# Rorisis/Co-Occ

Hardware: AMD Instinct MI355X
Metric: samples/sec (6-cam frame + sweep -> occ+render), 200x200x16 grid (higher is better)
Workload: dtype f32 (split-f16 products, fp32 accumulate)

## Files before the change

### co_occ_amd/_lib.py

```python
import ctypes
import os
import threading
import time

import torch

_HERE = os.path.dirname(os.path.abspath(__file__))
LIB_PATH = os.path.join(_HERE, "libcoocc_hip.so")

c_int, c_float, c_void_p, c_size_t, c_int64 = (ctypes.c_int, ctypes.c_float, ctypes.c_void_p,
                                               ctypes.c_size_t, ctypes.c_int64)


class ConvDesc(ctypes.Structure):
    _fields_ = [(n, c_void_p) for n in ("in_", "w", "out", "scale", "bias", "res", "gather", "out_rows", "ws")] + \
               [("ws_floats", c_int64)] + \
               [(n, c_int) for n in ("M", "Cin", "Cout", "taps", "in_stride", "out_stride", "res_stride",
                                     "B", "Xi", "Yi", "Zi", "Xo", "Yo", "Zo", "ksize", "stride", "pad",
                                     "relu", "res_mode", "splitk", "tile_hint", "kx", "ky", "kz", "px", "py", "pz",
                                     "wgroup_rows", "mfma_dtype")] + [("alpha", ctypes.c_float), ("M_dev", c_void_p), ("gather_stride", c_int), ("out16", c_void_p), ("out16_stride", c_int), ("out_h2", c_int),
                                                                   ("out_h2_twin", c_void_p), ("tile_sem", c_void_p), ("tile_sem_ints", c_int),
                                                                  ("alpha_dev", c_void_p), ("sx", c_int), ("sy", c_int), ("sz", c_int)]


class SearchDesc(ctypes.Structure):
    _fields_ = [("cat4", c_void_p), ("pts", c_void_p), ("pts_rows", c_int), ("pts_stride", c_int)] + \
               [(n, c_int) for n in ("C", "X", "Y", "Z", "K", "fps_num", "max_cluster")] + \
               [("radius", ctypes.c_float), ("dist_thresh", ctypes.c_float), ("offsets", c_void_p), ("noff", c_int)] + \
               [(n, c_void_p) for n in ("lin", "counts", "near_img", "near_pts", "rows", "rows_p", "ws")] + \
               [("ws_bytes", ctypes.c_size_t), ("counts_host", c_void_p)]


P, I, F, Z, L = c_void_p, c_int, c_float, c_size_t, c_int64
SIGNATURES = {
    "coocc_last_error": (ctypes.c_char_p, []),
    "coocc_abi_version": (I, []),
    "coocc_device_cu_count": (I, [P]),
    "coocc_stream_create_cu_mask": (I, [P, I, P]),
    "coocc_stream_destroy": (I, [P]),
    "coocc_event_create": (I, [I, P]),
    "coocc_event_destroy": (I, [P]),
    "coocc_event_record": (I, [P, P]),
    "coocc_stream_wait_event": (I, [P, P]),
    "coocc_event_synchronize": (I, [P]),
    "coocc_event_query": (I, [P]),
    "coocc_event_elapsed_ms": (I, [P, P, P]),
    "coocc_ncdhw_to_ndhwc": (I, [P, P, I, I, I, I, I, P]),
    "coocc_rows_to_bf16": (I, [P, I, L, I, P, P]),
    "coocc_rows_to_h2": (I, [P, I, L, I, F, P, P]),
    "coocc_rows_to_h2_ex": (I, [P, I, L, I, F, P, P, P]),
    "coocc_rows_to_h2_gather": (I, [P, I, P, L, P, I, F, P, P]),
    "coocc_rows_to_f16": (I, [P, I, L, I, P, P]),
    "coocc_wino_input_h2": (I, [P, I, I, I, I, I, I, I, P, I, L, F, P]),
    "coocc_wino_input_h2_ex": (I, [P, I, I, I, I, I, I, I, P, I, L, F, P, P]),
    "coocc_ndhwc_to_ncdhw": (I, [P, P, I, I, I, I, I, P]),
    "coocc_fuser_prepare": (I, [P, P, P, P, P, I, I, I, P]),
    "coocc_fuser_prepare_rows": (I, [P, I, I, P, I, I, P, P, P, I, I, I, P]),
    "coocc_compact_flags": (I, [P, I, P, P, P, Z, P]),
    "coocc_compact_flags_ex": (I, [P, I, P, P, P, P, Z, P]),
    "coocc_lin_to_coords": (I, [P, I, I, I, I, P, P, P]),
    "coocc_furthest_point_sampling": (I, [I, I, I, P, P, P, P]),
    "coocc_fps_voxels_ws": (Z, [I, I, I]),
    "coocc_fps_voxels": (I, [P, I, I, I, I, I, P, P, Z, P]),
    "coocc_fps_voxels_pair": (I, [P, I, P, P, P, I, P, P, Z, I, I, I, I, P]),
    "coocc_ball_query": (I, [I, I, I, F, F, I, P, P, P, P]),
    "coocc_knn_topk": (I, [I, I, I, P, P, P, P, P]),
    "coocc_voxel_index_map": (I, [P, I, I, P, P]),
    "coocc_voxel_index_map_dev": (I, [P, I, P, I, P, P]),
    "coocc_fine_sample_voxel_dev": (I, [P, I, I, I, I, P, I, P, I, P, P, P, I, P]),
    "coocc_fine_sample_img_dev": (I, [P, I, I, I, I, P, P, L, P, P, I, I, P]),
    "coocc_fine_mlp_pre_dev": (I, [P, I, P, I, L, P, I, P, P, P, F, P, P, P, P, F, P, P, I, P, P]),
    "coocc_fine_fused": (I, [P, I, I, I, P, I, I, I, P, P, I, P, I, P, P, P, P, F, P, P, P, P, F, P, P, I, P, P, P]),
    "coocc_fine2_pack": (I, [P, P, I, P, P, P, P, P, P, P, P, P, P]),
    "coocc_fine2_h2": (I, [P, I, I, I, I, P, I, I, I, P, P, I, P, P, P, P, F, F, I, P, P, P, P]),
    "coocc_fine_sample_img_lin": (I, [P, I, I, I, I, P, P, I, I, I, P, P, I, I, P]),
    "coocc_scatter_fine_dev": (I, [P, L, P, I, I, I, P, P, I, I, I, F, P]),
    "coocc_scatter_fine_grouped": (I, [P, I, I, P, I, P, I, I, I, I, P, F, P, P]),
    "coocc_ball_query_voxels": (I, [I, F, F, I, I, I, I, P, P, P, P, P]),
    "coocc_knn_topk_voxels": (I, [I, I, I, I, I, I, P, P, P, P, I, P, P, P, P, P]),
    "coocc_knn_assign": (I, [I, I, I, I, F, P, P, P, P, P, P]),
    "coocc_knn_threshold": (I, [I, F, P, P, P, P]),
    "coocc_index_rows_i32": (I, [P, I, P, I, P, P]),
    "coocc_conv_pack_weights": (L, [P, I, I, I, I, P]),
    "coocc_conv_fwd": (I, [ctypes.POINTER(ConvDesc), P]),
    "coocc_fuser_search_ws": (Z, [ctypes.POINTER(SearchDesc)]),
    "coocc_fuser_search": (I, [ctypes.POINTER(SearchDesc), P, P]),
    "coocc_fuser_search_oneshot": (I, [I]),
    "coocc_lin_to_coords_dev": (I, [P, I, P, I, I, I, I, I, P, P]),
    "coocc_fps_voxels_pair_ok": (I, [I, I, I, I]),
    "coocc_fps_voxels_pair_dev": (I, [P, I, P, P, P, I, P, P, Z, I, P, I, I, I, I, I, P]),
    "coocc_knn_topk_voxels_dev": (I, [I, I, I, I, I, P, P, P, P, I, P, P, P, P, P, I, I, P]),
    "coocc_ball_query_voxels_dev": (I, [I, F, F, I, I, I, I, P, P, P, P, P, I, P]),
    "coocc_knn_assign_dev": (I, [I, I, I, I, F, P, P, P, P, P, P, I, I, P]),
# ... 331 lines not shown
```

### co_occ_amd/core.py

```python
import ctypes

import torch

from . import _lib
from ._lib import TIMER, ConvDesc, KernelTimer, call, ptr

_F32 = torch.float32


TILE_HINT = int(__import__("os").environ.get("COOCC_CONV_TILE", "0"))
CONV_V2 = int(__import__("os").environ.get("COOCC_CONV_V2", "1"))
WINO = int(__import__("os").environ.get("COOCC_WINO", "1"))
WINO_MIN_ROWS = int(__import__("os").environ.get("COOCC_WINO_MIN_ROWS", "8192"))
CONV_PERSIST = __import__("os").environ.get("COOCC_CONV_PERSIST", "1") != "0"
ZTRIM = __import__("os").environ.get("COOCC_ZTRIM", "1") != "0"
WINO_TILE = int(__import__("os").environ.get("COOCC_WINO_TILE", "4"))
CONV_DTYPE = __import__("os").environ.get("COOCC_CONV_DTYPE", "f32")
CONV_ENGINE = __import__("os").environ.get("COOCC_CONV_ENGINE", "h2")
H2_WINO_SCALE = {2: 0.5, 3: 0.25, 4: 0.125}
H2_DIRECT = __import__("os").environ.get("COOCC_H2_DIRECT", "1") != "0"
INKERNEL_REDUCE = __import__("os").environ.get("COOCC_INKERNEL_REDUCE", "0") != "0"
H2_DIRECT_MIN_FLOPS = float(__import__("os").environ.get("COOCC_H2_MIN_FLOPS", "5e7"))


# ... 295 lines not shown
            return None
        return self._cached(("h2", ztrim), lambda: self._h2_layout(self._padded(self._taps(ztrim).double())))

    @staticmethod
    def _wino_G(tile):
        if tile == 2:
            return torch.tensor([[1., 0., 0.], [.5, .5, .5], [.5, -.5, .5], [0., 0., 1.]], dtype=torch.float64)
        if tile == 3:
            return torch.tensor([[1, 0, 0], [-2 / 9, 2 / 9, -2 / 9], [1 / 9, 2 / 9, 4 / 9], [-8 / 9, -4 / 9, -2 / 9], [0, 0, 1]],
                                dtype=torch.float64)
        return torch.tensor([[1, 0, 0], [1 / 3, 1 / 3, 1 / 3], [-1 / 3, 1 / 3, -1 / 3], [-16 / 15, -8 / 15, -4 / 15],
                             [1 / 15, -2 / 15, 4 / 15], [0, 0, 1]], dtype=torch.float64)

    def _wino_U(self, tile):
        G = self._wino_G(tile)
        w = self._w_raw.double().view(self.Cout, self.Cin, 3, 3, self.wino_kz)
        return torch.einsum("pa,qb,ncabz->pqncz", G, G, w).reshape(G.shape[0] ** 2, self.Cout, self.Cin, self.wino_kz)

    def wino_h2_pack(self, tile):
        return self._cached(("wino_h2", tile), lambda: torch.stack(
            [self._h2_layout(self._padded(u)) for u in self._wino_U(tile)], 0))

    def wino_pack(self, tile):
        def build():
            return torch.stack([lib_pack("coocc_conv_pack_weights", u, self.Cout, self.Cin, self.wino_kz, 0)
                                for u in self._wino_U(tile).float().contiguous()], 0)
        return self._cached(("wino", tile), build)


BF16_PRECONVERT = __import__("os").environ.get("COOCC_BF16_PRECONVERT", "1") != "0"
ZSHARE = __import__("os").environ.get("COOCC_BF16_ZSHARE", "1") != "0"

_stream_bufs = {}


def stream_buffer(device, kind, n, dtype=_F32, zero=False):
    key = (device.index, _lib.stream(device).value or 0, kind)
    t = _stream_bufs.get(key)
    if t is None or t.numel() < n:
        t = _stream_bufs[key] = (torch.zeros if zero else torch.empty)(n, device=device, dtype=dtype)
    return t


def stream_scratch(device, stream):
    h = stream.cuda_stream
    return [t for (d, s, _), t in _stream_bufs.items() if d == device.index and s == h]


def _wino_buffer(device, kind, nfloats):
    return stream_buffer(device, kind, nfloats, zero=True)


def scratch(device, kind, nfloats):
    return stream_buffer(device, "s:" + kind, nfloats)


def tile_sem(device, n=4096):
    return stream_buffer(device, "sem", n, torch.int32, zero=True)


def workspace(device, nfloats=64 << 20):
    return stream_buffer(device, "ws", nfloats)


def _lcm(a, b):
    import math
    return a * b // math.gcd(a, b)


# ... 375 lines not shown
```

### co_occ_amd/csrc/layout.hip

```cpp
#include <stdarg.h>
#include <stdlib.h>

#include "common.h"

typedef float f32x4 __attribute__((ext_vector_type(4)));

static thread_local char g_err[512] = "";

int coocc_set_error(int code, const char* fmt, ...) {
  va_list ap;
  va_start(ap, fmt);
  vsnprintf(g_err, sizeof(g_err), fmt, ap);
  va_end(ap);
  return code;
}

extern "C" const char* coocc_last_error(void) { return g_err; }
extern "C" int coocc_abi_version(void) { return 1; }

#define TV 64
#define TC 128

__global__ __launch_bounds__(256) void k_ncdhw_to_ndhwc(const float* __restrict__ src,
                                                         float* __restrict__ dst, int C, int V,
// ... 418 lines not shown
  if (cnt) {
    if (cnt[0] <= small_m || cnt[1] <= small_m) return;
    n = min(n, cnt[which]);
  }
  int i = blockIdx.x * blockDim.x + threadIdx.x;
  if (i >= n) return;
  int l = lin[i];
  int z = l % Z; l /= Z;
  int y = l % Y; l /= Y;
  int x = l % X; int b = l / X;
  if (xyz) { xyz[i * 3 + 0] = (float)x; xyz[i * 3 + 1] = (float)y; xyz[i * 3 + 2] = (float)z; }
  if (bxyz) { bxyz[i * 4 + 0] = b; bxyz[i * 4 + 1] = x; bxyz[i * 4 + 2] = y; bxyz[i * 4 + 3] = z; }
}

extern "C" int coocc_lin_to_coords(const int32_t* lin, int n, int X, int Y, int Z, float* xyz, int64_t* bxyz,
                                   void* stream) {
  COOCC_CHECK_ARG(lin && n >= 0 && X > 0 && Y > 0 && Z > 0, "lin_to_coords: bad args");
  if (n == 0) return COOCC_OK;
  hipLaunchKernelGGL(k_lin_to_coords, dim3(cdiv(n, 256)), dim3(256), 0, as_stream(stream), lin, n, X, Y, Z, xyz, bxyz,
                     (const int32_t*)nullptr, 0, 0);
  COOCC_LAUNCH_CHECK("k_lin_to_coords");
  return COOCC_OK;
}

extern "C" int coocc_lin_to_coords_dev(const int32_t* lin, int n_cap, const int32_t* cnt, int which, int small_m, int X, int Y, int Z,
                                       float* xyz, void* stream) {
  COOCC_CHECK_ARG(lin && xyz && cnt && n_cap > 0 && (unsigned)which < 2u && X > 0 && Y > 0 && Z > 0, "lin_to_coords_dev: bad args");
  hipLaunchKernelGGL(k_lin_to_coords, dim3(cdiv(n_cap, 256)), dim3(256), 0, as_stream(stream), lin, n_cap, X, Y, Z, xyz, (int64_t*)nullptr,
                     cnt, which, small_m);
  COOCC_LAUNCH_CHECK("k_lin_to_coords");
  return COOCC_OK;
}

extern "C" int coocc_device_cu_count(int* n) {
  COOCC_CHECK_ARG(n, "device_cu_count: null");
  int dev = 0;
  COOCC_HIP(hipGetDevice(&dev));
  hipDeviceProp_t prop;
  COOCC_HIP(hipGetDeviceProperties(&prop, dev));
  *n = prop.multiProcessorCount;
  return COOCC_OK;
}

extern "C" int coocc_stream_create_cu_mask(const uint32_t* mask_host, int nwords, void** stream_out) {
  COOCC_CHECK_ARG(mask_host && nwords > 0 && stream_out, "stream_create_cu_mask: bad args");
  hipStream_t s = nullptr;
  COOCC_HIP(hipExtStreamCreateWithCUMask(&s, (uint32_t)nwords, mask_host));
  *stream_out = (void*)s;
  return COOCC_OK;
}

extern "C" int coocc_stream_destroy(void* stream) {
  COOCC_CHECK_ARG(stream, "stream_destroy: null");
  COOCC_HIP(hipStreamDestroy(as_stream(stream)));
  return COOCC_OK;
}

extern "C" int coocc_event_create(int flags, void** event_out) {
  COOCC_CHECK_ARG(event_out && (flags & ~3) == 0, "event_create: bad args");
  hipEvent_t e = nullptr;
  COOCC_HIP(hipEventCreateWithFlags(&e, hipEventDisableSystemFence | ((flags & 1) ? 0u : hipEventDisableTiming) |
                                            ((flags & 2) ? hipEventBlockingSync : 0u)));
  *event_out = (void*)e;
  return COOCC_OK;
}
extern "C" int coocc_event_destroy(void* event) {
// ... 32 lines not shown
```

### co_occ_amd/csrc/search.hip

```cpp
#include <stdlib.h>
#include <string.h>

#include <atomic>

#include "common.h"

__global__ __launch_bounds__(256) void k_gather_xyz(const float* __restrict__ xyz, const int32_t* __restrict__ idx, int m,
                                                     float* __restrict__ out, const int32_t* __restrict__ cnt, int small_m) {
  if (cnt && (cnt[0] <= small_m || cnt[1] <= small_m)) return;
  const int i = blockIdx.x * blockDim.x + threadIdx.x;
  if (i >= m) return;
  const int s = idx[i];
  out[i * 3 + 0] = xyz[s * 3 + 0]; out[i * 3 + 1] = xyz[s * 3 + 1]; out[i * 3 + 2] = xyz[s * 3 + 2];
}

struct SearchWs {
  uint8_t* flags;
  int32_t* cws;
  float* xyz;
  int32_t* maps;
  int32_t* rep[2];
  float* rep_xyz[2];
  float* val[2];
  int32_t* nn[2];
// ... 74 lines not shown
  SRC(coocc_voxel_index_map_dev(lin_img, V, cnt, V, map_img, stream));
  SRC(coocc_voxel_index_map_dev(lin_pts, V, cnt + 1, V, map_pts, stream));
  if (!(sdiag & 1)) {
    const int rc = coocc_fps_voxels_pair_dev(lin_pts, 1, w.rep[0], w.fps[0], lin_img, 0, w.rep[1], w.fps[1], w.fps_bytes, V, cnt, m, X, Y, Z, m,
                                             stream);
    if (rc == 2) return coocc_set_error(COOCC_EINVAL, "fuser_search: the paired FPS refused a grid it had accepted");
    SRC(rc);
  }
  auto direction = [&](int dd, const int32_t* lin_q, int wq, const float* xyz_q, const int32_t* map_q, int wk, const float* xyz_k,
                       const int32_t* map_k, int32_t* near) -> int {
    if (sdiag & 2) return COOCC_OK;
    hipLaunchKernelGGL(k_gather_xyz, dim3(cdiv(m, 256)), dim3(256), 0, as_stream(stream), xyz_q, w.rep[dd], m, w.rep_xyz[dd], cnt, m);
    COOCC_LAUNCH_CHECK("k_gather_xyz");
    SRC(coocc_knn_topk_voxels_dev(m, K, X, Y, Z, w.rep[dd], lin_q, map_k, d->offsets, d->noff, w.rep_xyz[dd], xyz_k, w.val[dd], w.nn[dd], cnt,
                                  wk, m, stream));
    SRC(coocc_ball_query_voxels_dev(m, 0.f, d->radius, d->max_cluster, X, Y, Z, w.rep[dd], lin_q, map_q, w.group[dd], cnt, m, stream));
    SRC(coocc_knn_assign_dev(m, K, d->max_cluster, V, d->dist_thresh, w.val[dd], w.nn[dd], w.group[dd], w.winner[dd], near, cnt, wq, m, stream));
    return COOCC_OK;
  };
  SRC(direction(1, lin_img, 0, xyz_img, map_img, 1, xyz_pts, map_pts, d->near_pts));
  for (int k = 0; k < K && !(sdiag & 2); ++k)
    SRC(coocc_index_rows_i32_dev(K == 1 ? lin_pts : lin_img, K == 1 ? 1 : 0, d->near_pts, k, 0, V, d->rows_p + (size_t)k * V, cnt, m, stream));
  SRC(direction(0, lin_pts, 1, xyz_pts, map_pts, 0, xyz_img, map_img, d->near_img));
  for (int k = 0; k < K && !(sdiag & 2); ++k)
    SRC(coocc_index_rows_i32_dev(lin_img, 0, d->near_img, k, 1, V, d->rows + (size_t)k * V, cnt, m, stream));
  return COOCC_OK;
}

extern "C" int coocc_fuser_search(coocc_search_desc* d, void* stream, void* side_stream) {
  COOCC_CHECK_ARG(d && d->cat4 && d->pts && d->lin && d->counts && d->rows && d->rows_p && d->near_img && d->near_pts && d->ws &&
                      d->offsets && d->counts_host, "fuser_search: null pointer");
  COOCC_CHECK_ARG(d->C > 0 && d->X > 0 && d->Y > 0 && d->Z > 0 && d->K >= 1 && d->K <= 8 && d->fps_num > 0 && d->max_cluster > 0 &&
                      d->noff > 0, "fuser_search: bad sizes");
  COOCC_CHECK_ARG(stream != side_stream && side_stream, "fuser_search: needs a second stream for the img <- pts direction");
  const int V = d->X * d->Y * d->Z, K = d->K, C = d->C;
  SearchWs w = carve((char*)d->ws, V, K, d->fps_num, d->max_cluster, d->X, d->Y, d->Z);
  COOCC_CHECK_ARG(d->ws_bytes >= w.total, "fuser_search: workspace smaller than coocc_fuser_search_ws()");
  hipStream_t s0 = as_stream(stream), s1 = as_stream(side_stream);
  static const int sdiag = [] { const char* e = getenv("COOCC_SEARCH_DIAG_SKIP"); return e ? atoi(e) : 0; }();
  int32_t* lin_img = d->lin;
  int32_t* lin_pts = d->lin + V;

  SRC(coocc_fuser_prepare_rows(d->cat4, 1, 4 * C, d->pts, d->pts_rows, d->pts_stride, d->cat4, w.flags, w.flags + V, 1, C, V, stream));
  SRC(coocc_compact_flags(w.flags, V, lin_img, d->counts, w.cws, (size_t)(V / 1024 + 2) * 4, stream));
  SRC(coocc_compact_flags(w.flags + V, V, lin_pts, d->counts + 1, w.cws + (V / 1024 + 2), (size_t)(V / 1024 + 2) * 4, stream));
  if (oneshot_setting() && d->fps_num >= K && coocc_fps_voxels_pair_ok(V, d->X, d->Y, d->Z)) {
    const bool read = !((sdiag & 4) && d->counts_host[0] > 0);
    volatile int32_t* pin = read ? pinned_counts() : nullptr;
    if (read && !pin) return coocc_set_error(COOCC_ENOMEM, "fuser_search: no pinned host memory for the voxel counts");
    hipEvent_t got = nullptr;
    if (read) {
      static const bool fence = [] { const char* e = getenv("COOCC_SEARCH_COUNT_FENCE"); return e && e[0] == '1'; }();
      pin[0] = pin[1] = -1;
      COOCC_HIP(hipMemcpyAsync((void*)pin, d->counts, 8, hipMemcpyDeviceToHost, s0));
      COOCC_HIP(hipEventCreateWithFlags(&got, hipEventBlockingSync | hipEventDisableTiming | (fence ? 0u : hipEventDisableSystemFence)));
      if (hipEventRecord(got, s0) != hipSuccess) {
        (void)hipEventDestroy(got);
        return coocc_set_error(COOCC_EHIP, "fuser_search: recording the count event failed");
      }
    }
    const int rc = search_enqueue_dev(d, w, V, stream, sdiag);
    if (read) {
      const hipError_t e2 = hipEventSynchronize(got);
      (void)hipEventDestroy(got);
      if (e2 != hipSuccess) return coocc_set_error(COOCC_EHIP, "fuser_search: waiting for the voxel counts failed: %s", hipGetErrorString(e2));
      if (pin[0] < 0 || pin[1] < 0) {
        COOCC_HIP(hipStreamSynchronize(s0));
        if (pin[0] < 0 || pin[1] < 0) return coocc_set_error(COOCC_EHIP, "fuser_search: the voxel counts did not reach the host");
// ... 23 lines not shown
  int32_t* map_img = w.maps;
  int32_t* map_pts = w.maps + V;
  SRC(coocc_voxel_index_map(lin_img, Ni, V, map_img, stream));
  SRC(coocc_voxel_index_map(lin_pts, Np, V, map_pts, stream));

  const int pair_rc = (sdiag & 1) ? COOCC_OK
                                  : coocc_fps_voxels_pair(lin_pts, Np, w.rep[0], w.fps[0], lin_img, Ni, w.rep[1], w.fps[1], w.fps_bytes, d->X, d->Y,
                                                          d->Z, d->fps_num, stream);
  if (pair_rc != COOCC_OK && pair_rc != 2) return pair_rc;
  const bool paired = pair_rc == COOCC_OK;
  hipEvent_t fork = nullptr, join = nullptr;
  COOCC_HIP(hipEventCreateWithFlags(&fork, hipEventDisableTiming | hipEventDisableSystemFence));
  if (hipEventCreateWithFlags(&join, hipEventDisableTiming | hipEventDisableSystemFence) != hipSuccess) {
    (void)hipEventDestroy(fork);
    return coocc_set_error(COOCC_EHIP, "fuser_search: hipEventCreate failed");
  }
  bool forked = false;
  auto finish = [&](int rc) -> int {
    if (forked) {
      if (hipEventRecord(join, s1) != hipSuccess || hipStreamWaitEvent(s0, join, 0) != hipSuccess) {
        if (rc == COOCC_OK) rc = coocc_set_error(COOCC_EHIP, "fuser_search: joining the side stream failed");
      }
    }
    (void)hipEventDestroy(fork);
    (void)hipEventDestroy(join);
    return rc;
  };
#define SRF(call)                                \
  do {                                           \
    int rc__ = (call);                           \
    if (rc__ != COOCC_OK) return finish(rc__);   \
  } while (0)
  void* side_q = paired ? stream : side_stream;
  if (!paired) {
    if (hipEventRecord(fork, s0) != hipSuccess || hipStreamWaitEvent(s1, fork, 0) != hipSuccess)
      return finish(coocc_set_error(COOCC_EHIP, "fuser_search: forking the side stream failed"));
    forked = true;
  }

  auto direction = [&](int dd, void* st, const int32_t* lin_q, int Q, const float* xyz_q, const int32_t* map_q, int Nk,
                       const float* xyz_k, const int32_t* map_k, int32_t* near) -> int {
    if (sdiag & 2) return COOCC_OK;
    if (!paired) SRC(coocc_fps_voxels(lin_q, Q, d->X, d->Y, d->Z, d->fps_num, w.rep[dd], w.fps[dd], w.fps_bytes, st));
    hipLaunchKernelGGL(k_gather_xyz, dim3(cdiv(d->fps_num, 256)), dim3(256), 0, as_stream(st), xyz_q, w.rep[dd], d->fps_num, w.rep_xyz[dd],
                       (const int32_t*)nullptr, 0);
    COOCC_LAUNCH_CHECK("k_gather_xyz");
    SRC(coocc_knn_topk_voxels(d->fps_num, Nk, K, d->X, d->Y, d->Z, w.rep[dd], lin_q, map_k, d->offsets, d->noff, w.rep_xyz[dd], xyz_k,
                              w.val[dd], w.nn[dd], st));
    SRC(coocc_ball_query_voxels(d->fps_num, 0.f, d->radius, d->max_cluster, d->X, d->Y, d->Z, w.rep[dd], lin_q, map_q, w.group[dd], st));
    SRC(coocc_knn_assign(d->fps_num, K, d->max_cluster, Q, d->dist_thresh, w.val[dd], w.nn[dd], w.group[dd], w.winner[dd], near, st));
    return COOCC_OK;
  };
  SRF(direction(1, side_q, lin_img, Ni, xyz_img, map_img, Np, xyz_pts, map_pts, d->near_pts));
  for (int k = 0; k < K && !(sdiag & 2); ++k)
    SRF(coocc_index_rows_i32(K == 1 ? lin_pts : lin_img, K == 1 ? Np : Ni, d->near_pts + (size_t)k * Ni, Ni, d->rows_p + (size_t)k * V, side_q));
  SRF(direction(0, stream, lin_pts, Np, xyz_pts, map_pts, Ni, xyz_img, map_img, d->near_img));
  for (int k = 0; k < K && !(sdiag & 2); ++k)
    SRF(coocc_index_rows_i32(lin_img, Ni, d->near_img + (size_t)k * Np, Np, d->rows + (size_t)k * V, stream));
#undef SRF
  return finish(COOCC_OK);
}
```

### co_occ_amd/fuser.py

```python
import torch
from torch import nn

from . import _lib, streams
from ._lib import call, ptr
from . import core as _core_mod
from .core import PackCache, PackedConv, Rows, conv_rows, gather_conv_rows
from .registry import FUSION_LAYERS

_I32, _F32, _I64 = torch.int32, torch.float32, torch.int64


_side = {}


def _side_stream(dev, cur, which=0):
    key = (dev.index, cur.cuda_stream, which)
    if key not in _side:
        _side[key] = streams.side_stream_for(cur, which) or torch.cuda.Stream(device=dev, priority=getattr(cur, "priority", 0))
    return _side[key]


FPS_HIGH_PRIORITY = __import__("os").environ.get("COOCC_FPS_HIGH_PRIORITY", "0") != "0"
_fps_hi = {}
FPS_MAX_BUCKETS = 8 * 1024
# ... 311 lines not shown
                base, nbase = (lin_pts, Np) if K == 1 else (lin_img, Ni)
                for k in range(K):
                    call("coocc_index_rows_i32", ptr(base), nbase, ptr(sr.near_pts[k]), Ni, ptr(sr.rows_p[k]))
                sr.done_side = streams.new_event()
                sr.done_side.record()
            sr.near_img = _fps_nn_xyz(xyz_pts, xyz_img, q_lin=lin_pts if vox else None, k_lin=lin_img if vox else None, grid=vox,
                                      which=0, home=cur, **kw)
            sr.rows = slot.rows[:, :Np] if slot is not None else torch.empty(K, Np, device=dev, dtype=_I32)
            for k in range(K):
                call("coocc_index_rows_i32", ptr(lin_img), Ni, ptr(sr.near_img[k]), Np, ptr(sr.rows[k]))
            sr.keep = (xyz, lin, img, pts)
        elif Np or Ni:
            raise IndexError("BiFuser_N: one modality has no non-empty voxel (the reference fails on empty keys)")
        sr.done_main = streams.new_event()
        sr.done_main.record()
        return sr

    def search_native(self, pts_voxel_feats, slot):
        import ctypes
        X, Y, Z = slot.grid
        dev = slot.cat4.device
        pts_r = _as_rows_view(pts_voxel_feats)
        B = pts_r.B if pts_r is not None else pts_voxel_feats.shape[0]
        if B != 1 or (X + 3) // 4 * ((Y + 3) // 4) * ((Z + 7) // 8) > FPS_MAX_BUCKETS:
            return self.search(slot.img_rows().as_ncdhw(), pts_voxel_feats, slot=slot)
        d, _, host, _ = slot.native_desc()
        if pts_r is not None:
            d.pts, d.pts_rows, d.pts_stride = pts_r.t.data_ptr() + 4 * pts_r.coff, 1, pts_r.stride
            keep = pts_r.t
        else:
            keep = pts_voxel_feats.float().contiguous()
            d.pts, d.pts_rows, d.pts_stride = keep.data_ptr(), 0, 0
        cur = torch.cuda.current_stream(dev)
        side = _side_stream(dev, cur)
        rc = _lib.load().coocc_fuser_search(ctypes.byref(d), ctypes.c_void_p(cur.cuda_stream), ctypes.c_void_p(side.cuda_stream))
        if rc == 1:
            return self.search(slot.img_rows().as_ncdhw(), pts_voxel_feats, slot=slot)
        _lib.check(rc)
        Ni, Np = int(host[0]), int(host[1])
        self.last_counts = (Ni, Np)
        K, V = self.knum, slot.V
        sr = SearchResult(Rows(slot.cat4, 1, X, Y, Z, 4 * self.in_channels), slot.lin[0, :Ni], slot.lin[1, :Np])
        sr.slot = slot
        sr.near_img = slot.near[0, :K * Np].view(K, Np)
        sr.near_pts = slot.near[1, :K * Ni].view(K, Ni)
        sr.rows, sr.rows_p = slot.rows[:, :Np], slot.rows_p[:, :Ni]
        sr.keep = (keep,)
        sr.done_main = streams.new_event()
        sr.done_main.record()
        sr.done_side = sr.done_main
        return sr

    def finish(self, sr):
        cat4 = sr.cat4.t
        dev = cat4.device
        C = self.in_channels
        cur = torch.cuda.current_stream(dev)
        packs = self._packed()
        sr.done_main.wait(cur)
        for t in sr.tensors():
            t.record_stream(cur)
        if sr.rows is not None and sr.slot is not None:
            sr.done_side.wait(cur)
            self.finish_static(sr.slot)
            self.last_near = (sr.near_img, sr.near_pts)
        elif sr.rows is not None:
            sr.done_side.wait(cur)
            h2 = self._g1_h2(cat4, packs)
# ... 114 lines not shown
```

### co_occ_amd/serving.py

```python
import collections
import os
import threading
import time
from concurrent.futures import ThreadPoolExecutor

import torch

from . import core, graph as cg, streams as cstreams_

CAM_KEYS = ("rots", "trans", "intrins", "post_rots", "post_trans", "bda")


def _tensors_of(obj):
    if torch.is_tensor(obj):
        yield obj
    elif isinstance(obj, dict):
        for v in obj.values():
            yield from _tensors_of(v)
    elif isinstance(obj, (list, tuple)):
        for v in obj:
            yield from _tensors_of(v)


class Ticket:

    __slots__ = ("pipe", "index", "slot", "frame", "search", "out", "done", "copy", "events", "fallback", "ready", "pts_vol", "stream")

    def __init__(self, pipe, index, slot, frame, copy):
        self.pipe, self.index, self.slot, self.frame, self.copy = pipe, index, slot, frame, copy
        self.search = self.out = self.done = self.events = self.pts_vol = self.stream = None
        self.fallback = False
        self.ready = cstreams_.new_event()
        self.ready.record(torch.cuda.current_stream(pipe.dev))

    def result(self, wait=True):
        self.pipe._issue_through(self.index)
        if wait:
            self.done.synchronize()
            core.check_h2_overflow()
        return self.out


_DIAG_SKIP = int(os.environ.get("COOCC_SERVING_DIAG_SKIP", "0"))
SLOT_WAIT_HOST = os.environ.get("COOCC_SLOT_WAIT", "host") != "device"


def _clone_frame_item(v):
    if torch.is_tensor(v):
        return v.detach().clone()
    if isinstance(v, (list, tuple)):
        return type(v)(_clone_frame_item(x) for x in v)
    return v


class ServingPipeline:

    def __init__(self, model, example, slots=6, dense_streams=3, ahead=0, render=None, search_priority=0, after_replay=None,
                 time_dense=False, after_done=None):
        assert not model.training, "ServingPipeline serves the eval-mode (folded-BN) path"
        self.model = model
        pts = example.get("pts")
        if pts is None:
            with torch.no_grad():
                pts = model.extract_pts_feat(example["points"])[0]
        self.dev = dev = pts.device
        _, _, X, Y, Z = pts.shape
        self.grid = (X, Y, Z)
        self.render = (X >= 100 and Y >= 100 and Z >= 8 and model.use_rendering) if render is None else render
        self.n = n = max(1, int(slots))
        self.ndense = max(1, min(int(dense_streams), max(1, n - 1)))
        most = max(1, n - self.ndense) if n > 1 else 1
        self.ahead = most if ahead <= 0 else max(1, min(int(ahead), most))
        self.after_replay, self.after_done, self.time_dense = after_replay, after_done, time_dense
        self.dense_streams = [torch.cuda.Stream(device=dev) for _ in range(self.ndense)]
        self.search_streams = [torch.cuda.Stream(device=dev, priority=search_priority) for _ in range(n)]
        self.slots = [cg.make_slot(model, self.grid, dev) for _ in range(n)]
        self.static = [self._make_static(example) for _ in range(n)]
        self.slot_done = [None] * n
        self.graphs = [None] * n
        self.tpool = ThreadPoolExecutor(self.ahead)
        self.fallbacks = 0
        self.dense_ev = []
        self.trace = [] if os.environ.get("COOCC_SERVING_TRACE", "0") == "1" else None
        self._lock = threading.Lock()
        self._pending = collections.deque()
        self._queue = collections.deque()
        self._submitted = self._issued = 0
        self._issued_of_slot = [0] * n
        self._dispatched_of_slot = [0] * n
        self._last_sr = [None] * n
        self._example = {k: _clone_frame_item(v) for k, v in example.items()}
        self.recaptures = 0
        self._capture(example)
        self._watch = core.WeightWatch(model)

    def _make_static(self, fr):
        dev = self.dev
        cams = fr.get("cams")
        tr = fr["transform"]
        size = tr[-1]
        size = tuple(int(v[0]) if torch.is_tensor(v) else int(v) for v in size)
        st = dict(img_feats=[torch.empty_like(fr["img_feats"][0], device=dev)],
                  cams=tuple(torch.empty_like(t, device=dev) for t in cams) if cams is not None else None,
                  transform=tuple(torch.empty_like(t, device=dev) if torch.is_tensor(t) else t for t in tr[:-1]) + (size,),
                  gemo=None)
        if cams is None:
            st["gemo"] = torch.empty_like(fr["gemo"], device=dev) if fr.get("gemo") is not None else None
        return st

    def _copy_in(self, k, fr):
        st = self.static[k]
        st["img_feats"][0].copy_(fr["img_feats"][0], non_blocking=True)
        if st["cams"] is not None:
            for d, s in zip(st["cams"], fr["cams"]):
                d.copy_(s, non_blocking=True)
        for d, s in zip(st["transform"][:-1], fr["transform"][:-1]):
            if torch.is_tensor(d):
                d.copy_(s, non_blocking=True)
        if st["gemo"] is not None:
            st["gemo"].copy_(fr["gemo"], non_blocking=True)

    def _mark(self, t, tag):
        if self.trace is not None:
            self.trace.append((t.index, tag, time.perf_counter()))

    def _search(self, t):
        k, fr = t.slot, t.frame
        torch.cuda.set_device(self.dev)
        self._mark(t, "search_begin")
        st = self.search_streams[k]
        with torch.cuda.stream(st), torch.no_grad():
            t.ready.wait(st)
            if self.slot_done[k] is not None:
                if SLOT_WAIT_HOST:
                    self.slot_done[k].synchronize()
                else:
                    self.slot_done[k].wait(st)
            if self.time_dense:
                e0 = cstreams_.new_event(timing=True)
                e0.record()
            for v in _tensors_of(fr):
                if v.is_cuda:
                    v.record_stream(st)
            diag = _DIAG_SKIP if t.index >= 0 else 0
            if not diag & 1:
                self._copy_in(k, fr)
            pts = fr.get("pts")
            if pts is None:
                pts = self.model.extract_pts_feat(fr["points"])[0]
            t.pts_vol = pts
            self._mark(t, "search_native")
            slot = self.slots[k]
            if diag & 6 and fr.get("depth") is not None and self._last_sr[k] is not None:
                if not diag & 2:
                    self.model.img_view_transformer.lift_splat(fr["depth"], fr["ctx"], cams=fr["cams"], out=slot.img_rows())
                if not diag & 4:
                    sr = self.model.occ_fuser.search_native(pts, slot)
                else:
                    sr = self._last_sr[k]
                    sr.done_main = cstreams_.new_event()
                    sr.done_main.record()
                    sr.done_side = sr.done_main
            elif fr.get("depth") is not None:
                sr = cg.search_into_slot(self.model, slot, fr["depth"], fr["ctx"], fr["cams"], pts)
                self._last_sr[k] = sr
            else:
                vol = fr["img_voxel_feats"]
                slot.img_rows().as_ncdhw().copy_(vol)
                sr = self.model.occ_fuser.search_native(pts, slot) if cg.NATIVE_SEARCH else \
                    self.model.occ_fuser.search(slot.img_rows().as_ncdhw(), pts, slot=slot)
            if self.time_dense:
                if sr.done_side is not None:
                    sr.done_side.wait(st)
                e1 = cstreams_.new_event(timing=True)
                e1.record()
                t.events = (e0, e1)
        self._mark(t, "search_end")
        return sr

    def _capture(self, example):
        for k in range(self.n):
            t = Ticket(self, -1, k, example, False)
            sr = self._search(t)
            ds = self.dense_streams[k % self.ndense]
            sr.done_main.wait(ds)
            if sr.done_side is not None:
                sr.done_side.wait(ds)
            self.graphs[k] = cg.DenseGraph(self.model, self.slots[k], self.static[k], ds, render=self.render).capture()
        torch.cuda.synchronize(self.dev)
        core.check_h2_overflow()

    def submit(self, frame, copy=False):
        if self._watch.changed():
            self._recapture()
        with self._lock:
            i = self._submitted
            self._submitted += 1
            t = Ticket(self, i, i % self.n, frame, copy)
            self._pending.append(t)
        self._pump()
        return t

    def _pump(self, block_until=None):
        while True:
            with self._lock:
                while self._pending and len(self._queue) < self.ahead:
                    t = self._pending[0]
                    if self._dispatched_of_slot[t.slot] > self._issued_of_slot[t.slot]:
                        break
                    self._pending.popleft()
                    self._dispatched_of_slot[t.slot] += 1
                    self._mark(t, "dispatch")
                    t.search = self.tpool.submit(self._search, t)
                    self._queue.append(t)
                head = self._queue[0] if self._queue else None
            if head is None:
                return
            must = block_until is not None and self._issued <= block_until
            if not (must or head.search.done()):
                return
            sr = head.search.result()
            self._mark(head, "issue_begin")
            self._issue(head, sr)
            self._mark(head, "issue_end")
            with self._lock:
                self._queue.popleft()
                self._issued += 1
                self._issued_of_slot[head.slot] += 1

    def _issue_through(self, index):
        if self._issued <= index:
            self._pump(block_until=index)
        assert self._issued > index

    def _issue(self, t, sr):
        k = t.slot
        ds = self.dense_streams[k % self.ndense]
        sr.done_main.wait(ds)
        if sr.done_side is not None:
            sr.done_side.wait(ds)
        with torch.cuda.stream(ds), torch.no_grad():
            if self.time_dense:
                e0 = cstreams_.new_event(timing=True)
                e0.record()
            g = self.graphs[k]
            if g.fits(sr.counts):
                out = g.replay()
            else:
                self.fallbacks += 1
                t.fallback = True
                st = self.static[k]
                vf = self.model.occ_fuser(self.slots[k].img_rows().as_ncdhw(), t.pts_vol, search=sr)
                cam_geo = None
                if self.render and st["cams"] is not None:
                    cam_geo = self.model.img_view_transformer._camera_mats(*st["cams"])
                    cam_geo = (cam_geo[0].reshape(-1, cam_geo[0].shape[-1]),) + tuple(cam_geo[1:])
                out = self.model.decode(vf, st["gemo"], st["img_feats"], st["transform"], self.render, cam_geo=cam_geo)
            if self.time_dense:
                e1 = cstreams_.new_event(timing=True)
                e1.record()
                self.dense_ev.append((e0, e1, t.index, t.events))
            if t.copy:
                out = {kk: (v.clone() if torch.is_tensor(v) else (v.as_ncdhw().clone() if isinstance(v, core.Rows) else v))
                       for kk, v in out.items()}
            if self.after_replay is not None:
                self.after_replay(out)
            ev = cstreams_.new_event(blocking=True)
            ev.record()
        self.slot_done[k] = ev
        if self.after_done is not None:
            self.after_done(out, ev)
        t.out, t.done, t.stream = out, ev, ds
        t.frame = t.pts_vol = None
# ... 36 lines not shown
```

### include/coocc_hip.h

```cpp
#ifndef COOCC_HIP_H
#define COOCC_HIP_H

#include <stddef.h>
#include <stdint.h>

#ifdef __cplusplus
extern "C" {
#endif

#define COOCC_OK 0
#define COOCC_EINVAL (-1)
#define COOCC_EHIP (-2)
#define COOCC_ENOMEM (-3)

const char* coocc_last_error(void);
int coocc_abi_version(void);

int coocc_device_cu_count(int* n);
int coocc_stream_create_cu_mask(const uint32_t* mask_host, int nwords, void** stream_out);
int coocc_stream_destroy(void* stream);

int coocc_event_create(int flags, void** event_out);
int coocc_event_destroy(void* event);
int coocc_event_record(void* event, void* stream);
int coocc_stream_wait_event(void* stream, void* event);
int coocc_event_synchronize(void* event);
int coocc_event_query(void* event);
int coocc_event_elapsed_ms(void* start, void* stop, float* ms);


int coocc_ncdhw_to_ndhwc(const float* src, float* dst, int B, int C, int V, int dst_stride,
                         int dst_coff, void* stream);
int coocc_ndhwc_to_ncdhw(const float* src, float* dst, int B, int C, int V, int src_stride,
                         int src_coff, void* stream);

int coocc_fuser_prepare(const float* img, const float* pts, float* cat4, uint8_t* flag_img,
                        uint8_t* flag_pts, int B, int C, int V, void* stream);
int coocc_fuser_prepare_rows(const float* img, int img_rows, int img_stride, const float* pts, int pts_rows,
                             int pts_stride, float* cat4, uint8_t* flag_img, uint8_t* flag_pts, int B, int C, int V,
                             void* stream);

int coocc_compact_flags(const uint8_t* flags, int total, int32_t* lin, int32_t* count, void* ws,
                        size_t ws_bytes, void* stream);
int coocc_compact_flags_ex(const uint8_t* flags, int total, int32_t* lin, int32_t* count, int32_t* map, void* ws,
                           size_t ws_bytes, void* stream);
int coocc_lin_to_coords(const int32_t* lin, int n, int X, int Y, int Z, float* xyz, int64_t* bxyz,
                        void* stream);


int coocc_furthest_point_sampling(int b, int n, int m, const float* points, float* temp,
                                  int32_t* idx, void* stream);

size_t coocc_fps_voxels_ws(int X, int Y, int Z);
int coocc_fps_voxels(const int32_t* lin, int n, int X, int Y, int Z, int m, int32_t* idx, void* ws,
                     size_t ws_bytes, void* stream);
int coocc_fps_voxels_pair(const int32_t* lin0, int n0, int32_t* idx0, void* ws0, const int32_t* lin1, int n1, int32_t* idx1,
                          void* ws1, size_t ws_bytes_each, int X, int Y, int Z, int m, void* stream);

int coocc_ball_query(int b, int n, int m, float min_radius, float max_radius, int nsample,
                     const float* new_xyz, const float* xyz, int32_t* idx, void* stream);

#define COOCC_SEARCH_SMALL 1
typedef struct coocc_search_desc {
  float* cat4;
  const float* pts;
  int pts_rows, pts_stride;
  int C, X, Y, Z, K;
  int fps_num, max_cluster;
  float radius, dist_thresh;
  const uint32_t* offsets;
  int noff;
  int32_t* lin;
  int32_t* counts;
  int32_t* near_img;
  int32_t* near_pts;
  int32_t* rows;
  int32_t* rows_p;
  void* ws;
  size_t ws_bytes;
  int32_t* counts_host;
// ... 513 lines not shown
```

Before: 272.3.

## Run search on dense-stream lanes and batch frame input copies into one kernel

```diff
diff --git a/co_occ_amd/_lib.py b/co_occ_amd/_lib.py
--- a/co_occ_amd/_lib.py
+++ b/co_occ_amd/_lib.py
@@ -30,6 +30,12 @@
                [(n, c_void_p) for n in ("lin", "counts", "near_img", "near_pts", "rows", "rows_p", "ws")] + \
                [("ws_bytes", ctypes.c_size_t), ("counts_host", c_void_p)]
 
+
+class CopyItem(ctypes.Structure):
+    _fields_ = [("dst", c_void_p), ("src", c_void_p), ("bytes", ctypes.c_size_t)]
+
+
+COPY_MANY_MAX = 16
 
 P, I, F, Z, L = c_void_p, c_int, c_float, c_size_t, c_int64
 SIGNATURES = {
@@ -59,6 +65,7 @@
     "coocc_compact_flags": (I, [P, I, P, P, P, Z, P]),
     "coocc_compact_flags_ex": (I, [P, I, P, P, P, P, Z, P]),
     "coocc_lin_to_coords": (I, [P, I, I, I, I, P, P, P]),
+    "coocc_copy_many": (I, [P, I, P]),
     "coocc_furthest_point_sampling": (I, [I, I, I, P, P, P, P]),
     "coocc_fps_voxels_ws": (Z, [I, I, I]),
     "coocc_fps_voxels": (I, [P, I, I, I, I, I, P, P, Z, P]),
diff --git a/co_occ_amd/core.py b/co_occ_amd/core.py
--- a/co_occ_amd/core.py
+++ b/co_occ_amd/core.py
@@ -351,9 +351,25 @@
 ZSHARE = __import__("os").environ.get("COOCC_BF16_ZSHARE", "1") != "0"
 
 _stream_bufs = {}
+_scratch_ns = __import__("threading").local()
+
+
+class scratch_space:
+
+    def __init__(self, name):
+        self.name = name
+
+    def __enter__(self):
+        self.prev = getattr(_scratch_ns, "name", "")
+        _scratch_ns.name = self.name
+        return self
+
+    def __exit__(self, *exc):
+        _scratch_ns.name = self.prev
 
 
 def stream_buffer(device, kind, n, dtype=_F32, zero=False):
+    kind = getattr(_scratch_ns, "name", "") + kind
     key = (device.index, _lib.stream(device).value or 0, kind)
     t = _stream_bufs.get(key)
     if t is None or t.numel() < n:
diff --git a/co_occ_amd/csrc/layout.hip b/co_occ_amd/csrc/layout.hip
--- a/co_occ_amd/csrc/layout.hip
+++ b/co_occ_amd/csrc/layout.hip
@@ -474,6 +474,73 @@
   return COOCC_OK;
 }
 
+constexpr int COPY_THREADS = 256;
+constexpr unsigned long long COPY_CHUNK = 16384;
+constexpr unsigned long long COPY_MAX_BLOCKS = 4096;
+
+struct CopyTable {
+  char* dst[COOCC_COPY_MANY_MAX];
+  const char* src[COOCC_COPY_MANY_MAX];
+  unsigned long long bytes[COOCC_COPY_MANY_MAX];
+  unsigned first[COOCC_COPY_MANY_MAX + 1];
+  unsigned long long chunk;
+  int n;
+};
+
+__global__ __launch_bounds__(COPY_THREADS) void k_copy_many(const CopyTable t) {
+  const unsigned b = blockIdx.x;
+  int i = 0;
+#pragma unroll
+  for (int k = 1; k < COOCC_COPY_MANY_MAX; ++k)
+    if (k < t.n && b >= t.first[k]) i = k;
+  const unsigned long long off = (unsigned long long)(b - t.first[i]) * t.chunk;
+  const unsigned long long total = t.bytes[i];
+  if (off >= total) return;
+  const unsigned long long len = total - off < t.chunk ? total - off : t.chunk;
+  char* d = t.dst[i] + off;
+  const char* s = t.src[i] + off;
+  const uintptr_t al = (uintptr_t)d | (uintptr_t)s;
+  unsigned long long done = 0;
+  if ((al & 15) == 0) {
+    const unsigned long long nv = len >> 4;
+    for (unsigned long long v = threadIdx.x; v < nv; v += COPY_THREADS) ((uint4*)d)[v] = ((const uint4*)s)[v];
+    done = nv << 4;
+  }
+  if ((al & 3) == 0) {
+    const unsigned long long nw = (len - done) >> 2;
+    for (unsigned long long w = threadIdx.x; w < nw; w += COPY_THREADS) ((uint32_t*)(d + done))[w] = ((const uint32_t*)(s + done))[w];
+    done += nw << 2;
+  }
+  for (unsigned long long k = done + threadIdx.x; k < len; k += COPY_THREADS) d[k] = s[k];
+}
+
+extern "C" int coocc_copy_many(const coocc_copy_item* items, int n, void* stream) {
+  COOCC_CHECK_ARG(items && n >= 1 && n <= COOCC_COPY_MANY_MAX, "copy_many: 1 .. %d items per call", COOCC_COPY_MANY_MAX);
+  CopyTable t;
+  unsigned long long total = 0;
+  for (int i = 0; i < n; ++i) {
+    COOCC_CHECK_ARG(items[i].bytes == 0 || (items[i].dst && items[i].src), "copy_many: null pointer in item %d", i);
+    total += items[i].bytes;
+  }
+  if (total == 0) return COOCC_OK;
+  t.chunk = COPY_CHUNK * ((total / COPY_MAX_BLOCKS + COPY_CHUNK - 1) / COPY_CHUNK);
+  if (t.chunk < COPY_CHUNK) t.chunk = COPY_CHUNK;
+  unsigned nblk = 0;
+  for (int i = 0; i < COOCC_COPY_MANY_MAX; ++i) {
+    const bool on = i < n;
+    t.dst[i] = on ? (char*)items[i].dst : nullptr;
+    t.src[i] = on ? (const char*)items[i].src : nullptr;
+    t.bytes[i] = on ? (unsigned long long)items[i].bytes : 0ull;
+    t.first[i] = nblk;
+    nblk += (unsigned)((t.bytes[i] + t.chunk - 1) / t.chunk);
+  }
+  t.first[COOCC_COPY_MANY_MAX] = nblk;
+  t.n = n;
+  hipLaunchKernelGGL(k_copy_many, dim3(nblk), dim3(COPY_THREADS), 0, as_stream(stream), t);
+  COOCC_LAUNCH_CHECK("k_copy_many");
+  return COOCC_OK;
+}
+
 extern "C" int coocc_device_cu_count(int* n) {
   COOCC_CHECK_ARG(n, "device_cu_count: null");
   int dev = 0;
diff --git a/co_occ_amd/csrc/search.hip b/co_occ_amd/csrc/search.hip
--- a/co_occ_amd/csrc/search.hip
+++ b/co_occ_amd/csrc/search.hip
@@ -130,8 +130,9 @@
                       d->offsets && d->counts_host, "fuser_search: null pointer");
   COOCC_CHECK_ARG(d->C > 0 && d->X > 0 && d->Y > 0 && d->Z > 0 && d->K >= 1 && d->K <= 8 && d->fps_num > 0 && d->max_cluster > 0 &&
                       d->noff > 0, "fuser_search: bad sizes");
-  COOCC_CHECK_ARG(stream != side_stream && side_stream, "fuser_search: needs a second stream for the img <- pts direction");
   const int V = d->X * d->Y * d->Z, K = d->K, C = d->C;
+  COOCC_CHECK_ARG(side_stream ? stream != side_stream : coocc_fps_voxels_pair_ok(V, d->X, d->Y, d->Z) == 1,
+                  "fuser_search: needs a second stream for the img <- pts direction");
   SearchWs w = carve((char*)d->ws, V, K, d->fps_num, d->max_cluster, d->X, d->Y, d->Z);
   COOCC_CHECK_ARG(d->ws_bytes >= w.total, "fuser_search: workspace smaller than coocc_fuser_search_ws()");
   hipStream_t s0 = as_stream(stream), s1 = as_stream(side_stream);
@@ -221,6 +222,7 @@
     if (rc__ != COOCC_OK) return finish(rc__);   \
   } while (0)
   void* side_q = paired ? stream : side_stream;
+  if (!paired && !side_stream) return finish(coocc_set_error(COOCC_EINVAL, "fuser_search: needs a second stream for the img <- pts direction"));
   if (!paired) {
     if (hipEventRecord(fork, s0) != hipSuccess || hipStreamWaitEvent(s1, fork, 0) != hipSuccess)
       return finish(coocc_set_error(COOCC_EHIP, "fuser_search: forking the side stream failed"));
diff --git a/co_occ_amd/fuser.py b/co_occ_amd/fuser.py
--- a/co_occ_amd/fuser.py
+++ b/co_occ_amd/fuser.py
@@ -367,8 +367,9 @@
             keep = pts_voxel_feats.float().contiguous()
             d.pts, d.pts_rows, d.pts_stride = keep.data_ptr(), 0, 0
         cur = torch.cuda.current_stream(dev)
-        side = _side_stream(dev, cur)
-        rc = _lib.load().coocc_fuser_search(ctypes.byref(d), ctypes.c_void_p(cur.cuda_stream), ctypes.c_void_p(side.cuda_stream))
+        lib = _lib.load()
+        side = None if lib.coocc_fps_voxels_pair_ok(slot.V, X, Y, Z) == 1 else _side_stream(dev, cur).cuda_stream
+        rc = lib.coocc_fuser_search(ctypes.byref(d), ctypes.c_void_p(cur.cuda_stream), ctypes.c_void_p(side))
         if rc == 1:
             return self.search(slot.img_rows().as_ncdhw(), pts_voxel_feats, slot=slot)
         _lib.check(rc)
diff --git a/co_occ_amd/serving.py b/co_occ_amd/serving.py
--- a/co_occ_amd/serving.py
+++ b/co_occ_amd/serving.py
@@ -1,4 +1,5 @@
 import collections
+import ctypes
 import os
 import threading
 import time
@@ -6,7 +7,7 @@
 
 import torch
 
-from . import core, graph as cg, streams as cstreams_
+from . import _lib, core, graph as cg, streams as cstreams_
 
 CAM_KEYS = ("rots", "trans", "intrins", "post_rots", "post_trans", "bda")
 
@@ -43,6 +44,8 @@
 
 _DIAG_SKIP = int(os.environ.get("COOCC_SERVING_DIAG_SKIP", "0"))
 SLOT_WAIT_HOST = os.environ.get("COOCC_SLOT_WAIT", "host") != "device"
+SEARCH_LANES = os.environ.get("COOCC_SEARCH_LANES", "1") != "0"
+COPY_MANY = os.environ.get("COOCC_COPY_MANY", "1") != "0"
 
 
 def _clone_frame_item(v):
@@ -56,7 +59,7 @@
 class ServingPipeline:
 
     def __init__(self, model, example, slots=6, dense_streams=3, ahead=0, render=None, search_priority=0, after_replay=None,
-                 time_dense=False, after_done=None):
+                 time_dense=False, after_done=None, search_lanes=None):
         assert not model.training, "ServingPipeline serves the eval-mode (folded-BN) path"
         self.model = model
         pts = example.get("pts")
@@ -70,12 +73,14 @@
         self.n = n = max(1, int(slots))
         self.ndense = max(1, min(int(dense_streams), max(1, n - 1)))
         most = max(1, n - self.ndense) if n > 1 else 1
-        self.ahead = most if ahead <= 0 else max(1, min(int(ahead), most))
+        self.lanes = SEARCH_LANES if search_lanes is None else bool(search_lanes)
+        self.ahead = (1 if self.lanes else most) if ahead <= 0 else max(1, min(int(ahead), most))
         self.after_replay, self.after_done, self.time_dense = after_replay, after_done, time_dense
         self.dense_streams = [torch.cuda.Stream(device=dev) for _ in range(self.ndense)]
-        self.search_streams = [torch.cuda.Stream(device=dev, priority=search_priority) for _ in range(n)]
+        self.search_streams = None if self.lanes else [torch.cuda.Stream(device=dev, priority=search_priority) for _ in range(n)]
         self.slots = [cg.make_slot(model, self.grid, dev) for _ in range(n)]
         self.static = [self._make_static(example) for _ in range(n)]
+        self._copy_tables = [None] * n
         self.slot_done = [None] * n
         self.graphs = [None] * n
         self.tpool = ThreadPoolExecutor(self.ahead)
@@ -110,15 +115,33 @@
 
     def _copy_in(self, k, fr):
         st = self.static[k]
-        st["img_feats"][0].copy_(fr["img_feats"][0], non_blocking=True)
+        pairs = [(st["img_feats"][0], fr["img_feats"][0])]
         if st["cams"] is not None:
-            for d, s in zip(st["cams"], fr["cams"]):
-                d.copy_(s, non_blocking=True)
-        for d, s in zip(st["transform"][:-1], fr["transform"][:-1]):
-            if torch.is_tensor(d):
-                d.copy_(s, non_blocking=True)
+            pairs += zip(st["cams"], fr["cams"])
+        pairs += [(d, s) for d, s in zip(st["transform"][:-1], fr["transform"][:-1]) if torch.is_tensor(d)]
         if st["gemo"] is not None:
-            st["gemo"].copy_(fr["gemo"], non_blocking=True)
+            pairs.append((st["gemo"], fr["gemo"]))
+        tab = self._copy_tables[k]
+        if tab is None:
+            tab = self._copy_tables[k] = (_lib.CopyItem * len(pairs))()
+            for it, (d, _) in zip(tab, pairs):
+                it.dst, it.bytes = d.data_ptr(), d.numel() * d.element_size()
+        direct = [COPY_MANY and torch.is_tensor(s) and s.device == d.device and s.dtype == d.dtype and s.shape == d.shape
+                  and s.is_contiguous() and d.is_contiguous() for d, s in pairs]
+        if not all(direct):
+            for (d, s), ok in zip(pairs, direct):
+                if not ok:
+                    d.copy_(s, non_blocking=True)
+            pairs = [p for p, ok in zip(pairs, direct) if ok]
+            tab = (_lib.CopyItem * max(1, len(pairs)))()
+            for it, (d, _) in zip(tab, pairs):
+                it.dst, it.bytes = d.data_ptr(), d.numel() * d.element_size()
+        for it, (_, s) in zip(tab, pairs):
+            it.src = s.data_ptr()
+        lib, stream = _lib.load(), _lib.stream(self.dev)
+        for i in range(0, len(pairs), _lib.COPY_MANY_MAX):
+            m = min(_lib.COPY_MANY_MAX, len(pairs) - i)
+            _lib.check(lib.coocc_copy_many(ctypes.byref(tab, i * ctypes.sizeof(_lib.CopyItem)), m, stream))
 
     def _mark(self, t, tag):
         if self.trace is not None:
@@ -128,10 +151,10 @@
         k, fr = t.slot, t.frame
         torch.cuda.set_device(self.dev)
         self._mark(t, "search_begin")
-        st = self.search_streams[k]
-        with torch.cuda.stream(st), torch.no_grad():
+        st = self.dense_streams[k % self.ndense] if self.lanes else self.search_streams[k]
+        with torch.cuda.stream(st), torch.no_grad(), core.scratch_space("search%d:" % k if self.lanes else ""):
             t.ready.wait(st)
-            if self.slot_done[k] is not None:
+            if self.slot_done[k] is not None and not self.lanes:
                 if SLOT_WAIT_HOST:
                     self.slot_done[k].synchronize()
                 else:
@@ -170,7 +193,7 @@
                 sr = self.model.occ_fuser.search_native(pts, slot) if cg.NATIVE_SEARCH else \
                     self.model.occ_fuser.search(slot.img_rows().as_ncdhw(), pts, slot=slot)
             if self.time_dense:
-                if sr.done_side is not None:
+                if sr.done_side is not None and sr.done_side is not sr.done_main:
                     sr.done_side.wait(st)
                 e1 = cstreams_.new_event(timing=True)
                 e1.record()
@@ -178,14 +201,19 @@
         self._mark(t, "search_end")
         return sr
 
+    def _after_search(self, sr, ds):
+        if self.lanes and sr.done_side is sr.done_main:
+            return
+        sr.done_main.wait(ds)
+        if sr.done_side is not None and sr.done_side is not sr.done_main:
+            sr.done_side.wait(ds)
+
     def _capture(self, example):
         for k in range(self.n):
             t = Ticket(self, -1, k, example, False)
             sr = self._search(t)
             ds = self.dense_streams[k % self.ndense]
-            sr.done_main.wait(ds)
-            if sr.done_side is not None:
-                sr.done_side.wait(ds)
+            self._after_search(sr, ds)
             self.graphs[k] = cg.DenseGraph(self.model, self.slots[k], self.static[k], ds, render=self.render).capture()
         torch.cuda.synchronize(self.dev)
         core.check_h2_overflow()
@@ -236,9 +264,7 @@
     def _issue(self, t, sr):
         k = t.slot
         ds = self.dense_streams[k % self.ndense]
-        sr.done_main.wait(ds)
-        if sr.done_side is not None:
-            sr.done_side.wait(ds)
+        self._after_search(sr, ds)
         with torch.cuda.stream(ds), torch.no_grad():
             if self.time_dense:
                 e0 = cstreams_.new_event(timing=True)
diff --git a/include/coocc_hip.h b/include/coocc_hip.h
--- a/include/coocc_hip.h
+++ b/include/coocc_hip.h
@@ -46,6 +46,14 @@
                            size_t ws_bytes, void* stream);
 int coocc_lin_to_coords(const int32_t* lin, int n, int X, int Y, int Z, float* xyz, int64_t* bxyz,
                         void* stream);
+
+#define COOCC_COPY_MANY_MAX 16
+typedef struct coocc_copy_item {
+  void* dst;
+  const void* src;
+  size_t bytes;
+} coocc_copy_item;
+int coocc_copy_many(const coocc_copy_item* items, int n, void* stream);
 
 
 int coocc_furthest_point_sampling(int b, int n, int m, const float* points, float* temp,
```

Result: faster. 300.7, median of 6 (+10.4%).
